# interactiveaudiolab/ppgs

Measured on AMD Instinct MI355X. Metric: PPG frames/sec (whole node), mel repr, batch=32x1000 frames, higher is better.
Workload: dtype bf16; 1 GPU; configs[1]: mel representation, batch=32 x 1000 frames per GPU, audio resident in HBM -> (32,40,1000) fp32 posteriors in HBM; batch=32, frames=1000, per_gpu_batches=1, parallelism=utterance-sharded x1, no data-path collective

## Files before the change

### ppgs_amd/csrc/ppg_engine.hip

```cpp
#include "ppg_pack.h"

#include <stdarg.h>

using namespace ppg;

static thread_local std::string g_error;

int ppg::fail_message(int code, const char* fmt, ...) {
    char buf[512];
    va_list ap;
    va_start(ap, fmt);
    vsnprintf(buf, sizeof(buf), fmt, ap);
    va_end(ap);
    g_error = buf;
    return code;
}

PpgEngine::~PpgEngine() {
    (void)hipSetDevice(device);
#ifdef PPG_TIMING_BUILD
    dump_timing_stamps(this);
#endif
    for (void* p : {(void*)d_overflow, (void*)head_dbg, (void*)ffn_dbg, (void*)attn_dbg, (void*)lin_dbg}) if (p) (void)hipFree(p);
    for (auto& kv : plans) if (kv.second->buf) (void)hipFree(kv.second->buf);
// ... 335 lines not shown
        HIP_OK(hipMemset(e->attn_dbg, 0, 512 + 4096 * 32));
    }
#endif
#ifdef PPG_H32_TIMING
    if (getenv("PPGS_AMD_H32_TIMING")) {
        HIP_OK(hipMalloc(reinterpret_cast<void**>(&e->head_dbg), 512));
        HIP_OK(hipMemset(e->head_dbg, 0, 512));
    }
#endif
#ifdef PPG_FFN_TIMING
    if (getenv("PPGS_AMD_FFN_TIMING")) {
        HIP_OK(hipMalloc(reinterpret_cast<void**>(&e->ffn_dbg), 2048));
        HIP_OK(hipMemset(e->ffn_dbg, 0, 2048));
    }
#endif
    if (e->ffn_nt < 0 || e->ffn_nt > 3) e->ffn_nt = 0;
    {
        hipDeviceProp_t prop;
        if (hipGetDeviceProperties(&prop, device) == hipSuccess && prop.multiProcessorCount > 0)
            e->num_cus = prop.multiProcessorCount;
    }

    int rc;
    if ((rc = pk.upload_f32(wts->position_encoding, (size_t)cfg->max_positions * H, 0, &e->pe))) return rc;
    {
        const float* w = wts->input_weight;
        const int Cp = e->Cp;
        rc = pk.matrix(H, 5 * Cp, H, e->in_total_groups * e->KG,
                       [&](int row, int k) { const int h = pair_row(row), tap = k / Cp, c = k % Cp; return c < C ? w[((size_t)h * C + c) * 5 + tap] : 0.f; },
                       &e->w_in);
        if (rc) return rc;
        if ((rc = pk.upload_f32(wts->input_bias, H, 0, &e->b_in))) return rc;
    }
    const int RB = H / 128, KS = H / 16;
    auto wave_row = [&](int w, int rb, int ln) { return 32 * RB * w + 32 * rb + phi(ln & 31); };
    if (e->head32) {
        const float* w = wts->input_weight;
        const int KSI = 5 * e->Cp / 16, frags = 4 * RB * KSI;
        rc = pk.image(frags + 1, [&](int f, int ln, int j) {
            if (f >= frags) return 0.f;
            const int ks = f % KSI, rb = (f / KSI) % RB, wv = f / (KSI * RB);
            const int tap = ks / (e->Cp / 16), c = frag_k(ks % (e->Cp / 16), ln, j);
            return c < C ? w[((size_t)wave_row(wv, rb, ln) * C + c) * 5 + tap] : 0.f;
        }, &e->win_img);
        if (rc) return rc;
    }
    {
        const float* w = wts->output_weight;
        rc = pk.matrix(cfg->output_channels, 5 * H, 48, e->out_total_groups * e->KG,
                       [&](int n, int k) { const int tap = k / H, c = k % H; return w[((size_t)n * H + c) * 5 + tap]; },
                       &e->w_out);
        if (rc) return rc;
        if ((rc = pk.upload_f32(wts->output_bias, cfg->output_channels, 48, &e->b_out))) return rc;
    }
    e->layers.resize(L);
    const float qscale = (float)(1.4426950408889634 / sqrt((double)dh));
    std::vector<float> in_w((size_t)3 * H * H), in_b((size_t)3 * H);
    for (int l = 0; l < L; ++l) {
        DevLayer& d = e->layers[l];
        for (size_t i = 0; i < in_w.size(); ++i) in_w[i] = wts->in_proj_weight[l][i] * (i < (size_t)H * H ? qscale : 1.0f);
        for (int i = 0; i < 3 * H; ++i) in_b[i] = wts->in_proj_bias[l][i] * (i < H ? qscale : 1.0f);
        const float *wq = in_w.data(), *wo = wts->out_proj_weight[l], *w1 = wts->linear1_weight[l], *w2 = wts->linear2_weight[l];
        auto paired = [&](const float* w, int rows, int cols, bool pair_rows, bool pair_k, char** dst) {
            return pk.matrix(rows, cols, rows, cols, [&](int r, int c) { return w[(size_t)(pair_rows ? pair_row(r) : r) * cols + (pair_k ? pair_row(c) : c)]; }, dst);
        };
        if ((rc = paired(wq, 3 * H, H, true, false, &d.wqkv))) return rc;
        if ((rc = paired(wo, H, H, true, false, &d.wo))) return rc;
        if ((rc = paired(w1, F, H, false, false, &d.w1))) return rc;
        if ((rc = paired(w2, H, F, true, false, &d.w2))) return rc;
        d.wqkvk = d.wqkv;
        d.w1k = d.w1;
        if (pk.fmt == Fmt::F32) {
            if ((rc = paired(wq, 3 * H, H, true, true, &d.wqkvk))) return rc;
            if ((rc = paired(w1, F, H, false, true, &d.w1k))) return rc;
        }
        {
            const bool bf = pk.fmt != Fmt::F32;
            rc = pk.matrix(H, F, H, F,
                           [&](int row, int c) {
                               const int r = pair_row(row);
                               if (!bf) return w2[(size_t)r * F + c];
                               const int grp = c / 32, s = c % 32, g = s / 8, ee = (s % 8) / 4, rr = s % 4;
                               return w2[(size_t)r * F + grp * 32 + 16 * ee + 4 * g + rr];
                           },
                           &d.w2p);
            if (rc) return rc;
        }
        auto qkv_row = [&](int w, int st, int ln) {
            const int rb = st % RB, kind = st / RB;
            return kind < 2 ? kind * H + wave_row(w, rb, ln) : 2 * H + pair_row(32 * RB * w + 32 * rb + (ln & 31));
        };
        if (e->layer32) {
            rc = pk.image(4 * RB * KS, [&](int f, int ln, int j) {
                const int ks = f % KS, rb = (f / KS) % RB, w = f / (KS * RB);
                return wo[(size_t)wave_row(w, rb, ln) * H + frag_k(ks, ln, j)];
            }, &d.wo_img);
            if (rc) return rc;
            rc = pk.image(F / 128 * 4 * KS, [&](int f, int ln, int j) {
                const int ks = f % KS, w = (f / KS) & 3, ch = f / (KS * 4);
                return w1[(size_t)(ch * 128 + 32 * w + (ln & 31)) * H + panel_k(ks, ln, j)];
            }, &d.w1_img);
            if (rc) return rc;
            rc = pk.image(F / 128 * 4 * RB * 8, [&](int f, int ln, int j) {
                const int ks = f & 7, rb = (f >> 3) % RB, w = (f / (8 * RB)) & 3, ch = f / (8 * RB * 4);
                return w2[(size_t)wave_row(w, rb, ln) * F + ch * 128 + hidden_k(ks, ln, j)];
            }, &d.w2_img);
// ... 218 lines not shown
        if (r.form[l] == kLayer32) {
            Timed t(e, PPG_K_FFN, r.s);
            Layer32Args a{};
            a.ao = r.ao; a.wo_img = d.wo_img; a.w1_img = d.w1_img; a.w2_img = d.w2_img;
            a.bo = d.bo; a.g1 = d.g1; a.e1 = d.e1; a.b1 = d.b1; a.b2 = d.b2; a.g2 = d.g2; a.e2 = d.e2;
            a.X = r.X; a.Xb = r.Xb; a.M = M; a.F = F; a.H = H; a.dbg = l == 0 ? e->ffn_dbg : nullptr;
            a.debug_mode = e->l32_debug;
            a.x_half = e->x16;
            a.sub_tiles = r.sub32;
            a.write_x = l + 1 < c.num_layers;
            if (qkv_next) {
                qkv_tail(&a, r, e->layers[l + 1].wq_img, e->layers[l + 1].bqkv);
                a.Xb = nullptr;
            }
            LAUNCH_OK(ppg::launch_layer32(prec, a, r.s), "layer32");
            return PPG_OK;
        }
        if (!r.fuse_op && !(r.form[l] == kFfn32x2 && e->ffn32x2 >= 2)) {
            Timed t(e, PPG_K_OUTPROJ_LN, r.s);
            LinearArgs a = outproj_ln_args(e, rows, d, r.ao);
            if (l == 0 && e->lin_dbg_class == PPG_K_OUTPROJ_LN) a.dbg = e->lin_dbg;
            LAUNCH_OK(ppg::launch_linear(prec, EPI_RESLN, H / 16, r.lnt_ln, a, 1, r.s), "out-proj+LN");
        }
        Timed t(e, PPG_K_FFN, r.s);
        if (r.form[l] == kFfn32x2) {
            Ffn32X2Args a{};
            a.xb = r.Xb; a.X = r.X; a.xb_out = r.Xb; a.w1_img = d.w1x_img; a.w2_img = d.w2x_img;
            a.b1 = d.b1; a.b2 = d.b2; a.g2 = d.g2; a.e2 = d.e2; a.M = M; a.F = F; a.H = H;
            if (e->ffn32x2 >= 2) { a.ao = r.ao; a.wo_img = d.wox_img; a.bo = d.bo; a.g1 = d.g1; a.e1 = d.e1; }
            a.dbg = l == 0 ? e->ffn_dbg : nullptr;
            if (qkv_next) qkv_tail(&a, r, e->layers[l + 1].wqx_img, e->layers[l + 1].bqkv);
            LAUNCH_OK(ppg::launch_ffn32x2(a, r.s), "ffn32x2");
        } else if (r.form[l] == kFfnFused) {
            FfnArgs a = ffn_args(e, rows, d, r.ws.ffn_splits, reinterpret_cast<float*>(r.base + r.ws.part));
            a.dbg = l == 0 ? e->ffn_dbg : nullptr;
            if (r.fuse_op) ffn_fuse_outproj(&a, d, r.ao);
            if (qkv_next) ffn_fuse_qkv(&a, rows, e->layers[l + 1], r.qk, r.vt, r.ws.vt_ld);
            LAUNCH_OK(ppg::launch_ffn(prec, a, r.ws.ffn_nt, r.s), "ffn");
        } else {
            LinearArgs a = gemm_args(e, rows, r.act_x, H, d.w1, d.b1, F);
            a.out_rows = r.hid; a.out_ld = F;
            LAUNCH_OK(ppg::launch_linear(prec, EPI_RELU, 16, r.lnt, a, F / 256, r.s), "ffn1");
            LinearArgs b = gemm_args(e, rows, r.hid, F, d.w2, d.b2, H);
            b.gamma = d.g2; b.beta = d.e2;
            LAUNCH_OK(ppg::launch_linear(prec, EPI_RESLN, H / 16, r.lnt_ln, b, 1, r.s), "ffn2+LN");
        }
        return PPG_OK;
    };

    auto enqueue_outconv = [&](const Route& r) -> int {
        Timed t(e, PPG_K_OUTCONV_SOFTMAX, r.s);
        LinearArgs a = outconv_args(e, rows_of(r), r.act_x, out, frames, softmax);
        if (e->lin_dbg_class == PPG_K_OUTCONV_SOFTMAX) a.dbg = e->lin_dbg;
        if (e->outconv && ppg::outconv_supported(prec, a)) LAUNCH_OK(ppg::launch_outconv(prec, a, r.s), "out-conv+softmax");
        else LAUNCH_OK(ppg::launch_linear(prec, EPI_OUTCONV, 3, r.lnt_ln, a, 1, r.s), "out-conv+softmax");
        return PPG_OK;
    };

    std::vector<Route> routes;
    routes.reserve(plan.groups.size());
    for (size_t gi = 0; gi < plan.groups.size(); ++gi) routes.push_back(route_of(plan.groups[gi], gi == 0 ? s : e->side_streams[gi - 1]));
    return fork_join(s, e->ev_fork, e->side_streams.data(), e->ev_join.data(), routes.size() - 1, [&]() -> int {
        for (int seg = 0; seg < c.num_layers + 2; ++seg)
            for (const Route& r : routes) {
                const int rc = seg == 0 ? enqueue_head(r) : seg <= c.num_layers ? enqueue_layer(r, seg - 1) : enqueue_outconv(r);
                if (rc) return rc;
            }
        return PPG_OK;
    });
}

int ppg_engine_nonfinite(PpgEngine* e, int clear, int* flag) {
    if (!e || !flag) return fail(PPG_EINVAL, "null argument");
    if (!e->d_overflow) { *flag = 0; return PPG_OK; }
    std::lock_guard<std::mutex> lock(e->mu);
    HIP_OK(hipSetDevice(e->device));
    unsigned value = 0;
    HIP_OK(hipMemcpy(&value, e->d_overflow, sizeof(value), hipMemcpyDeviceToHost));
    if (value && clear) HIP_OK(hipMemset(e->d_overflow, 0, sizeof(value)));
    *flag = (int)value;
    return PPG_OK;
}

int ppg_engine_pipelines(const PpgEngine* e, int tokens) {
    if (!e || tokens < 0) return 0;
    return group_count(e, tokens);
}

int ppg_engine_profile(PpgEngine* e, int enable) {
    if (!e) return fail(PPG_EINVAL, "null engine");
    e->profiling = (unsigned)enable;
    if (enable) (void)hipSetDevice(e->device);
    for (int cls = 0; enable && cls < PPG_K_COUNT; ++cls) {
        if (!(e->profiling & (1u << cls))) continue;
        while (e->events[cls].size() < 32) {
            EventPair p;
            if (hipEventCreateWithFlags(&p.a, kTimingEventFlags) != hipSuccess || hipEventCreateWithFlags(&p.b, kTimingEventFlags) != hipSuccess) break;
            e->events[cls].push_back(p);
        }
    }
    return PPG_OK;
}

int ppg_engine_profile_reset(PpgEngine* e) {
    if (!e) return fail(PPG_EINVAL, "null engine");
    for (auto& u : e->events_used) u = 0;
    for (auto& q : e->launch_seq) q = 0;
// ... 17 lines not shown
```

### ppgs_amd/csrc/ppg_head32.hip

```cpp
#include "ppg_layer32.h"

namespace {

constexpr int HID = 256;
constexpr int CP = 96;
constexpr int ROWB = 208;
constexpr int HALO = 2;
constexpr int KSI = 5 * CP / 16;
constexpr int KSH = KSI / 2;

template <int K0, int TBN>
struct OffIn {
    static constexpr int at(int i) {
        const int ks = K0 + i / TBN, tb = i % TBN;
        return (32 * tb + ks / (CP / 16)) * ROWB + (ks % (CP / 16)) * 32;
    }
};

template <class P, int TBS>
__global__ __launch_bounds__(256) __attribute__((amdgpu_waves_per_eu(1, 1))) void head32_kernel(Head32Args a) {
    using G = Geo<HID, TBS>;
    constexpr int RB = G::RB, KS = G::KS, TB = G::TBN, TOKS = G::TOKS;
    constexpr int TBT = tile_blocks(HID);
    constexpr bool SUB = TBS != TBT;
    constexpr int NSUB = (TBT + TBS - 1) / TBS;
    static_assert(RB == 2 && KSI % 2 == 0, "two row blocks per wave, two register sets");
    extern __shared__ __attribute__((aligned(16))) char smem[];
    const int tid = threadIdx.x;
    if ((int)blockIdx.x >= a.tiles * NSUB) {
        for (int job = blockIdx.x - a.tiles * NSUB; job <= a.nwin + 1; job += gridDim.x - a.tiles * NSUB) {
            if (job == a.nwin + 1) {
                for (int i = tid; i < a.qk_slack_bytes / 16; i += 256) reinterpret_cast<uint4*>(a.qk_slack)[i] = make_uint4(0u, 0u, 0u, 0u);
            } else if (job == a.nwin) {
                const int chunks = (a.vt_ld - a.vt_tokens) * 2 / 16;
                for (int i = tid; i < a.vt_rows * chunks; i += 256) {
                    const int r = i / chunks, c = i - r * chunks;
                    *reinterpret_cast<uint4*>(a.vt_out + ((size_t)r * a.vt_ld + a.vt_tokens) * 2 + c * 16) = make_uint4(0u, 0u, 0u, 0u);
                }
            } else {
                const PpgWindow w = a.win[job];
                const int r16 = (w.frames + 15) & ~15, r32 = (w.frames + 31) & ~31;
                if (r32 != r16) {
                    const int col = w.vt_off + r32 - 32;
                    for (int i = tid; i < a.vt_rows * 4; i += 256) {
                        const int r = i >> 2, g = i & 3;
                        *reinterpret_cast<uint2*>(a.vt_out + ((size_t)r * a.vt_ld + col + 8 * g + 4) * 2) = make_uint2(0u, 0u);
                    }
                }
            }
        }
        return;
    }
    const int lane = tid & 63;
    const int wave = __builtin_amdgcn_readfirstlane(tid >> 6);
    const int tok = lane & 31, hh = lane >> 5;
    const int tile = SUB ? (int)blockIdx.x / NSUB : (int)blockIdx.x;
    const int tb0 = SUB ? ((int)blockIdx.x % NSUB) * TBS : 0;
    const int nblk = SUB ? min(TBS, TBT - tb0) : TBS;
    const int m0 = tile * (32 * TBT) + 32 * tb0;
    const uint32_t lds0 = lds_addr32(smem);
    const uint32_t voff = lane * 16;
    const uint32_t pb0 = lds0 + G::L_ACT + lane * 16;
    const int fbase = 32 * RB * wave;
    char* rows = smem + G::L_H;
    static_assert((TOKS + 2 * HALO) * ROWB <= TB * 8 * 1024, "the gathered tile fits the h region");
    float* bq_lds = reinterpret_cast<float*>(smem + G::L_BQ);

#ifdef PPG_H32_TIMING
    auto pstamp = [&](int k) {
        if (!SUB && a.dbg && blockIdx.x == 0 && lane == 0) a.dbg[wave * 16 + k] = __builtin_amdgcn_s_memtime();
    };
#else
    auto pstamp = [&](int) {};
#endif
    pstamp(0);
    u32x4 w1f[16], w2f[16];
    auto load16 = [&](u32x4 (&wf)[16], const char* base) {
        [&]<int... K>(std::integer_sequence<int, K...>) { (gload_frag<K>(wf[K], voff, base), ...); }(std::make_integer_sequence<int, 16>{});
    };
    const char* wimg = a.win_img + ((size_t)wave * RB * KSI) * 1024;
    const char* wq0 = a.wq_img + ((size_t)wave * 3 * RB * KS) * 1024;
    load16(w1f, wimg);
    load16(w2f, wimg + (size_t)KSI * 1024);

    if (tid < TOKS + 2 * HALO && !(PPG_DBG(a) & 4)) {
        const int m = m0 - HALO + tid;
        int frame = -1;
        size_t base = 0;
        if (m >= 0) {
            const TokMeta tm = tok_meta(a.blk_win, a.win, m, a.M);
            if (tm.w >= 0 && tm.tt < tm.frames) {
                const PpgWindow w = a.win[tm.w];
                frame = w.chunked ? max(w.start + tm.tt - a.overlap, 0) : tm.tt;
                base = (size_t)w.item * a.C * a.T;
            }
        }
        uint32_t* dst = reinterpret_cast<uint32_t*>(rows + tid * ROWB);
        const int C = a.C;
        const bool row_live = frame >= 0;
        const size_t off = base + (size_t)max(frame, 0);
        float v[CP];
        if (a.dtype == PPG_DTYPE_F16) {
            const __half* src = reinterpret_cast<const __half*>(a.feats) + off;
#pragma unroll
            for (int c = 0; c < CP; ++c) v[c] = __half2float(src[(size_t)min(c, C - 1) * a.T]);
// ... 18 lines not shown
        live[t] = tm.w >= 0 && tm.tt < tm.frames;
        valid[t] = live[t] && tm.tt < tm.valid;
        tt[t] = live[t] ? tm.tt : 0;
        dlo[t] = live[t] ? -tm.tt : -HALO;
        dhi[t] = live[t] ? tm.frames - 1 - tm.tt : HALO;
        unsigned bits = 0;
#pragma unroll
        for (int tap = 0; tap < 5; ++tap)
            if (__any(tap - HALO < dlo[t] || tap - HALO > dhi[t])) bits |= 1u << tap;
        edge[t] = bits;
    }

    pstamp(2);
    f32x16 yacc[RB][TB];
    const f32x16 zero = {0.f, 0.f, 0.f, 0.f, 0.f, 0.f, 0.f, 0.f, 0.f, 0.f, 0.f, 0.f, 0.f, 0.f, 0.f, 0.f};
    const uint32_t rb0 = lds0 + G::L_H + (uint32_t)(tok * ROWB + hh * 16);
    float4 pe[TB][4];
    auto load_pe = [&](int rb) {
#pragma unroll
        for (int t = 0; t < TB; ++t)
#pragma unroll
            for (int q = 0; q < 4; ++q)
                pe[t][q] = *reinterpret_cast<const float4*>(a.pe + (size_t)tt[t] * HID + fbase + 32 * rb + 16 * hh + 4 * q);
    };
    auto round = [&](auto r_tag, auto after_wait) {
        constexpr int R = decltype(r_tag)::value;
        vm_wait_all(w1f);
        vm_wait_all(w2f);
        after_wait();
        if constexpr (R == 0) __syncthreads();
        stream<OffIn<KSH * R, TB>, KSH * TB, 6>(rb0, rb0, [&](auto ic, const u32x4& bf) {
            constexpr int i = decltype(ic)::value;
            constexpr int ksl = i / TB, tb = i % TB, tap = (KSH * R + ksl) / (CP / 16);
            u32x4 b = bf;
            if constexpr (tap != HALO) {
                if (edge[tb] & (1u << tap)) {
                    const bool ok = tap - HALO >= dlo[tb] && tap - HALO <= dhi[tb];
                    b = u32x4{ok ? bf.x : 0u, ok ? bf.y : 0u, ok ? bf.z : 0u, ok ? bf.w : 0u};
                }
            }
            if constexpr (R == 0 && ksl == 0) {
                yacc[0][tb] = P::mma32(w1f[0], b, zero);
                yacc[1][tb] = P::mma32(w2f[0], b, zero);
            } else {
                yacc[0][tb] = P::mma32(w1f[ksl], b, yacc[0][tb]);
                yacc[1][tb] = P::mma32(w2f[ksl], b, yacc[1][tb]);
            }
            if constexpr (R == 0 && tb == TB - 1) {
                gload_frag<ksl>(w1f[ksl], voff, wimg + (size_t)KSH * 1024);
                gload_frag<ksl>(w2f[ksl], voff, wimg + (size_t)(KSI + KSH) * 1024);
            }
        });
    };
    if (!(PPG_DBG(a) & 1)) round(std::integral_constant<int, 0>{}, [] {});
    else __syncthreads();
    pstamp(3);
    if (!(PPG_DBG(a) & 1)) round(std::integral_constant<int, 1>{}, [&] { load_pe(0); });
    else load_pe(0);

    pstamp(4);
    float* xt = a.X + ((size_t)tile * 4 + wave) * (TBT * RB * 4 * 256) + lane * 4;
    char* xh = reinterpret_cast<char*>(a.X) + ((size_t)tile * 4 + wave) * (TBT * RB * 2 * 1024) + lane * 16;
    auto emit = [&](auto rb_tag) {
        constexpr int rb = decltype(rb_tag)::value;
        const int f0 = fbase + 32 * rb + 16 * hh;
        float4 bias[4], pv[TB][4];
#pragma unroll
        for (int q = 0; q < 4; ++q) bias[q] = *reinterpret_cast<const float4*>(a.b_in + f0 + 4 * q);
#pragma unroll
        for (int t = 0; t < TB; ++t)
#pragma unroll
            for (int q = 0; q < 4; ++q) pv[t][q] = pe[t][q];
        if constexpr (rb + 1 < RB) load_pe(rb + 1);
#pragma unroll
        for (int t = 0; t < TB; ++t) {
            f32x16 y;
#pragma unroll
            for (int q = 0; q < 4; ++q) {
                y[4 * q + 0] = live[t] ? pv[t][q].x + (valid[t] ? yacc[rb][t][4 * q + 0] + bias[q].x : 0.f) : 0.f;
                y[4 * q + 1] = live[t] ? pv[t][q].y + (valid[t] ? yacc[rb][t][4 * q + 1] + bias[q].y : 0.f) : 0.f;
                y[4 * q + 2] = live[t] ? pv[t][q].z + (valid[t] ? yacc[rb][t][4 * q + 2] + bias[q].z : 0.f) : 0.f;
                y[4 * q + 3] = live[t] ? pv[t][q].w + (valid[t] ? yacc[rb][t][4 * q + 3] + bias[q].w : 0.f) : 0.f;
                if (!a.x_half && t < nblk)
                    *reinterpret_cast<float4*>(xt + (((tb0 + t) * RB + rb) * 4 + q) * 256) = make_float4(y[4 * q + 0], y[4 * q + 1], y[4 * q + 2], y[4 * q + 3]);
            }
            if (a.x_half && t < nblk) {
#pragma unroll
                for (int s2 = 0; s2 < 2; ++s2)
                    *reinterpret_cast<u32x4*>(xh + (((tb0 + t) * RB + rb) * 2 + s2) * 1024) = u32x4{pack_f16x2(y[8 * s2 + 0], y[8 * s2 + 1]), pack_f16x2(y[8 * s2 + 2], y[8 * s2 + 3]),
                                                                                      pack_f16x2(y[8 * s2 + 4], y[8 * s2 + 5]), pack_f16x2(y[8 * s2 + 6], y[8 * s2 + 7])};
            }
            panel_store<P, HID, TBS>(pb0, wave, t, rb, y);
        }
    };
    emit(std::integral_constant<int, 0>{});
    emit(std::integral_constant<int, 1>{});
    pstamp(5);
    load16(w1f, wq0);
    vm_wait_all(w1f);
    pstamp(6);

    Layer32Args la{};
    la.wq_img = a.wq_img; la.qk_out = a.qk_out; la.vt_out = a.vt_out; la.vt_ld = a.vt_ld;
    la.blk_win = a.blk_win; la.win = a.win; la.M = a.M; la.H = HID;
    if (!(PPG_DBG(a) & 2)) qkv_tail<P, HID, TBS>(la, smem, m0, w1f, w2f, nblk);
    asm volatile("s_waitcnt vmcnt(0)" ::: "memory");
    pstamp(7);
}

}

namespace ppg {

hipError_t launch_head32(int precision, const Head32Args& a, hipStream_t s) {
    if (a.H != HID || a.C > CP || a.M <= 0 || a.tiles != (a.M + 32 * tile_blocks(HID) - 1) / (32 * tile_blocks(HID))) return hipErrorInvalidValue;
    auto launch = [&](auto kern, auto geo, int subs) {
        using G = decltype(geo);
        const size_t lds = G::L_B1;
        const dim3 grid(a.tiles * subs + std::min(a.nwin + 2, 32));
        static ppg::LdsLimit limit;
        const hipError_t e = limit.ensure(reinterpret_cast<const void*>(kern), lds);
        if (e != hipSuccess) return e;
        hipLaunchKernelGGL(kern, grid, dim3(256), lds, s, a);
        return hipGetLastError();
    };
    constexpr int T5 = tile_blocks(HID);
    if (precision == PPG_PRECISION_BF16) return a.sub_tiles ? launch(head32_kernel<PrecBF16, 2>, Geo<HID, 2>{}, 3) : launch(head32_kernel<PrecBF16, T5>, Geo<HID>{}, 1);
    if (precision == PPG_PRECISION_FP16) return a.sub_tiles ? launch(head32_kernel<PrecF16, 2>, Geo<HID, 2>{}, 3) : launch(head32_kernel<PrecF16, T5>, Geo<HID>{}, 1);
    return hipErrorInvalidValue;
}

}
```

### ppgs_amd/csrc/ppg_host.h

```cpp
#pragma once

#include "ppg_launch.h"

#include <limits.h>
#include <math.h>
#include <stdio.h>
#include <string.h>

#include <map>
#include <memory>
#include <mutex>
#include <string>
#include <vector>

namespace ppg {

int fail_message(int code, const char* fmt, ...);
inline int (&fail)(int, const char*, ...) = fail_message;

#define HIP_OK(expr) \
    do { if (hipError_t e_ = (expr); e_ != hipSuccess) return fail(PPG_EDEVICE, "%s failed: %s", #expr, hipGetErrorString(e_)); } while (0)
#define LAUNCH_OK(expr, what) \
    do { if (hipError_t he_ = (expr); he_ != hipSuccess) return fail(PPG_EDEVICE, "%s: %s", what, hipGetErrorString(he_)); } while (0)

// ... 105 lines not shown
    size_t xw, x, xb, qk, vt, ao, hid, part, total;
    int ffn_nt, ffn_splits;
    int vt_ld, qk_rows;
};

}

struct PpgEngine {
    PpgConfig cfg{};
    int device = 0;
    int sz = 4;
    int KG = 16;
    int Cp = 0;
    int in_groups_per_tap = 0, in_total_groups = 0;
    int out_groups_per_tap = 0, out_total_groups = 0;
    int head_dim = 0;
    int ffn_nt = 0;
    int lin_nt = 0;
    int num_cus = 256;
    bool ffn_fused = true;
    bool qkv_fused = true;
    int ffn_split_max = 0;
    int ffn_splits_forced = 0;
    bool ffn_mixed = true;
    bool op_fused = true;
    bool attn_xcd = true;
    bool outconv = true;
    bool head32 = true;
    char* win_img = nullptr;
    int attn_narrow = 1;
    unsigned* d_overflow = nullptr;
    int ffn32x2 = 3;
    bool subtile = true;
    bool x16 = false;
    bool layer32 = true;
    bool ffn_split = true;
    int num_streams = 2;
    std::vector<hipStream_t> side_streams;
    bool stream_one_pass = false;
    int stream_min_rows = 128;
    hipEvent_t ev_fork = nullptr;
    std::vector<hipEvent_t> ev_join;
    int l32_debug = 0, h32_debug = 0;
    unsigned long long* ffn_dbg = nullptr;
    unsigned long long* head_dbg = nullptr;
    unsigned long long* attn_dbg = nullptr;
    unsigned long long* lin_dbg = nullptr;
    int lin_dbg_class = -1;
    ppg::Packer pack;
    bool split() const { return pack.split(); }
    float* pe = nullptr;
    char* w_in = nullptr; float* b_in = nullptr;
    char* w_out = nullptr; float* b_out = nullptr;
    std::vector<ppg::DevLayer> layers;
    std::map<std::string, std::unique_ptr<ppg::DevPlan>> plans;
    uint64_t plan_stamp = 0;
    std::vector<ppg::RetiredBuf> retired;
    ppg::StageSlot stage[4];
    int stage_next = 0;
    std::mutex mu;
    unsigned profiling = 0;
    std::vector<ppg::EventPair> events[PPG_K_COUNT];
    size_t events_used[PPG_K_COUNT] = {0};
    int profile_stride = 1;
    size_t launch_seq[PPG_K_COUNT] = {0};

    ~PpgEngine();
};

namespace ppg {

#if defined(PPG_FFN_TIMING) || defined(PPG_ATTN_TIMING) || defined(PPG_H32_TIMING) || defined(PPG_LIN_TIMING)
#define PPG_TIMING_BUILD 1
void dump_timing_stamps(const PpgEngine* e);
#endif

int choose_nt(int num_cus, int forced_nt, int M, int max_nt);
inline int ffn_chunks(int hidden, int ffn, int sz) { return ffn / (32768 / (hidden * sz)); }
constexpr size_t kLdsBytes = 163840;
inline size_t ffn_lds_bytes(int hidden, int ffn, int rows) { return 131072 + (size_t)ffn * 4 + (size_t)rows * hidden * 4; }
inline bool ffn_fits(int hidden, int ffn, bool op) { return ffn_lds_bytes(hidden, ffn, op ? 9 : 6) <= kLdsBytes; }
inline bool ffn_mixed_fits(int hidden, int ffn) { return ffn_lds_bytes(hidden, ffn, 6) + 16384 <= kLdsBytes; }
Workspace layout(const PpgEngine* e, int tokens, int vt_tokens);
inline int stream_query_tile(int head_dim) { return head_dim == 128 ? attn_query_tile(head_dim) / 2 : attn_query_tile(head_dim); }

template <class Body>
int fork_join(hipStream_t s, hipEvent_t fork, const hipStream_t* side, const hipEvent_t* join, size_t n, Body&& body) {
    if (n == 0) return body();
    const int rc = [&]() -> int {
        HIP_OK(hipEventRecord(fork, s));
        for (size_t i = 0; i < n; ++i) HIP_OK(hipStreamWaitEvent(side[i], fork, 0));
        return body();
    }();
    if (rc != PPG_OK) {
        for (size_t i = 0; i < n; ++i) {
            (void)hipEventRecord(join[i], side[i]);
            (void)hipStreamWaitEvent(s, join[i], 0);
        }
        return rc;
    }
    for (size_t i = 0; i < n; ++i) {
        HIP_OK(hipEventRecord(join[i], side[i]));
        HIP_OK(hipStreamWaitEvent(s, join[i], 0));
    }
    return PPG_OK;
}
// ... 102 lines not shown
```

### ppgs_amd/csrc/ppg_launch.h

```cpp
#pragma once

#include <algorithm>
#include <cstdlib>
#include <hip/hip_runtime.h>

#include "ppg_device.h"

namespace ppg {

inline int env_switch(const char* name, int dflt) {
    const char* s = getenv(name);
    return s ? atoi(s) : dflt;
}
#ifdef PPG_EXPERIMENT_SWITCHES
inline int env_experiment(const char* name, int dflt) { return env_switch(name, dflt); }
inline bool env_experiment_set(const char* name) { return getenv(name) != nullptr; }
#else
inline int env_experiment(const char*, int dflt) { return dflt; }
inline bool env_experiment_set(const char*) { return false; }
#endif

int attn_query_tile(int head_dim);

hipError_t launch_gather(int precision, const GatherArgs& a, hipStream_t s);
hipError_t launch_fill(float* p, size_t n, float v, hipStream_t s);

hipError_t launch_linear(int precision, int epi, int nb, int nt, const LinearArgs& a, int ypasses, hipStream_t s);
constexpr int kFfnMixedTiling = 5;
hipError_t launch_ffn(int precision, const FfnArgs& a, int nt, hipStream_t s);
hipError_t launch_attn(int precision, const AttnArgs& a, int nitems, int heads, int head_dim, hipStream_t s);
hipError_t launch_layer32(int precision, const Layer32Args& a, hipStream_t s);
hipError_t launch_head32(int precision, const Head32Args& a, hipStream_t s);
hipError_t launch_gemm32(int precision, const Gemm32Args& a, hipStream_t s);
hipError_t launch_posconv(int precision, const PosConvArgs& a, int batch, hipStream_t s);
hipError_t launch_ffn32x2(const Ffn32X2Args& a, hipStream_t s);
int ffn32x2_tokens();
bool ffn32x2_supported(int H, int F);
bool outconv_supported(int precision, const LinearArgs& a);
hipError_t launch_outconv(int precision, const LinearArgs& a, hipStream_t s);
int layer32_tokens(int hidden);
int layer32_max_ffn(int hidden);
hipError_t launch_w2v2_layer0(int precision, const float* audio, int batch, long samples, long frames, int rows_per_item,
                              const float* w0, const float* gamma, const float* beta, double* moments, float2* scale_shift,
                              char* out, hipStream_t s);
hipError_t launch_w2v2_layernorm(int precision, int H, const float* in32, const char* in16, const float* gamma, const float* beta,
                                 long rows, int T_in, int R_out, float eps, float* out32, char* out16, hipStream_t s);
hipError_t launch_w2v2_output(int precision, const char* rows, int batch, int rows_per_item, long frames, float* out, hipStream_t s);

constexpr int kFrontendFrames = 16;
constexpr int kMelSteps = 8;
constexpr int kMelSegment = 5;

struct LdsLimit {
    size_t bytes[32] = {};
    hipError_t ensure(const void* kernel, size_t lds) {
        int device = 0;
        if (hipGetDevice(&device) != hipSuccess || device < 0 || device >= 32) device = 0;
        if (bytes[device] >= lds) return hipSuccess;
        const hipError_t e = hipFuncSetAttribute(kernel, hipFuncAttributeMaxDynamicSharedMemorySize, (int)lds);
        if (e == hipSuccess) bytes[device] = lds;
        return e;
    }
};

struct FrontendTables {
    const float* hann;
    const float2* twiddle;
    const void* mel_img;
    const int4* mel_prog;
    unsigned long long* dbg;
};

hipError_t launch_frontend(const FrontendTables& tb, const float* audio, int batch, int samples,
                           void* spec, void* mel, hipStream_t s);

struct FrontendStreamItem {
    int lo;
    int hi;
    int cbase;
    int split;
    int frames;
    int keep;
    int cur;
    int pad;
};
constexpr int kFrontendStreamItems = 64;
struct FrontendStreamArgs {
    const float* chunk;
    float* carry;
    long chunk_pitch;
    int cap;
    int item0;
// ... 8 lines not shown
```

### ppgs_amd/csrc/ppg_outconv.hip

```cpp
#include "ppg_lds.h"
#include "ppg_launch.h"

#include <utility>

#ifdef PPG_ONLY_BF16
#define PPG_OTHER_PRECISIONS 0
#else
#define PPG_OTHER_PRECISIONS 1
#endif

namespace {

constexpr int OT = 64;
constexpr int HALO = 2;
constexpr int NB = 3;
constexpr int KTAP = 256;
constexpr int KSTEPS = 5 * KTAP / 32;
constexpr int WROW = 5 * KTAP * 2;
constexpr int WP = WROW + 32;
constexpr int TP = KTAP * 2 + 32;
constexpr int L_TILE = NB * 16 * WP;
constexpr int LDS_BYTES = L_TILE + (OT + 2 * HALO) * TP;
static_assert(LDS_BYTES <= 160 * 1024, "one workgroup per CU");
constexpr int ROW_CHUNKS = KTAP * 2 / 16;
constexpr int STG = ((OT + 2 * HALO) * ROW_CHUNKS + 255) / 256;

template <class P>
__global__ __launch_bounds__(256) void outconv_kernel(LinearArgs a) {
    extern __shared__ __attribute__((aligned(16))) char smem[];
    const int tid = threadIdx.x;
    const int lane = tid & 63;
    const int wave = __builtin_amdgcn_readfirstlane(tid >> 6);
    const int idx = lane & 15, g = lane >> 4;

    float bias[NB][4];
#pragma unroll
    for (int nb = 0; nb < NB; ++nb) {
        const float4 bv = *reinterpret_cast<const float4*>(a.bias + nb * 16 + 4 * g);
        bias[nb][0] = bv.x; bias[nb][1] = bv.y; bias[nb][2] = bv.z; bias[nb][3] = bv.w;
    }

    const int ntiles = (a.M + OT - 1) / OT;
    u32x4 stg[STG];
    auto fetch = [&](int tile) {
#pragma unroll
        for (int j = 0; j < STG; ++j) {
            const int i = min(tid + 256 * j, (OT + 2 * HALO) * ROW_CHUNKS - 1);
            const int r = i / ROW_CHUNKS, piece = i - r * ROW_CHUNKS;
            const int m = min(max(tile * OT - HALO + r, 0), a.M - 1);
            stg[j] = *reinterpret_cast<const u32x4*>(a.act + (size_t)m * a.lda_bytes + piece * 16);
        }
    };
    auto stash = [&]() {
#pragma unroll
        for (int j = 0; j < STG; ++j) {
            const int i = tid + 256 * j;
            if (i < (OT + 2 * HALO) * ROW_CHUNKS) {
                const int r = i / ROW_CHUNKS, piece = i - r * ROW_CHUNKS;
                *reinterpret_cast<u32x4*>(smem + L_TILE + r * TP + piece * 16) = stg[j];
            }
        }
    };
    struct Meta { TokMeta tm; int keep_lo, keep_hi, out_frame, item; };
    auto lookup_block = [&](int tile) {
        const int m = tile * OT + 16 * wave + idx;
        return m < a.M ? a.blk_win[m >> 4] : -1;
    };
    auto lookup_window = [&](int tile, int w) {
        Meta r;
        const PpgWindow win = a.win[max(w, 0)];
        r.tm.w = w;
        r.tm.tt = w >= 0 ? tile * OT + 16 * wave + idx - win.tok_off : 0;
        r.tm.frames = w >= 0 ? win.frames : 0;
        r.tm.valid = w >= 0 ? win.valid : 0;
        r.keep_lo = win.keep_lo; r.keep_hi = win.keep_hi; r.out_frame = win.out_frame; r.item = win.item;
        return r;
    };
    Meta cur{};
    int wcur = -1;
    if ((int)blockIdx.x < ntiles) { fetch(blockIdx.x); wcur = lookup_block(blockIdx.x); }

    constexpr int WPIECES = NB * 16 * (WROW / 16), WBATCH = 15;
    static_assert(WPIECES == 2 * WBATCH * 256, "two batches");
#pragma unroll
    for (int half = 0; half < 2; ++half) {
        u32x4 wv[WBATCH];
#pragma unroll
        for (int j = 0; j < WBATCH; ++j) {
            const int i = tid + 256 * (half * WBATCH + j);
            const int row = i / (WROW / 16), piece = i - row * (WROW / 16);
            wv[j] = *reinterpret_cast<const u32x4*>(a.W + (size_t)row * a.total_groups * 64 + piece * 16);
        }
        if (half == 1 && (int)blockIdx.x < ntiles) cur = lookup_window(blockIdx.x, wcur);
#pragma unroll
        for (int j = 0; j < WBATCH; ++j) {
            const int i = tid + 256 * (half * WBATCH + j);
            const int row = i / (WROW / 16), piece = i - row * (WROW / 16);
            *reinterpret_cast<u32x4*>(smem + row * WP + piece * 16) = wv[j];
        }
    }
    const uint32_t lds0 = lds_addr(smem);
    uint32_t waddr[NB];
#pragma unroll
    for (int nb = 0; nb < NB; ++nb) waddr[nb] = lds0 + (uint32_t)((nb * 16 + idx) * WP + g * 16);
    const uint32_t xaddr = lds0 + (uint32_t)(L_TILE + (16 * wave + idx) * TP + g * 16);
    const int step = gridDim.x;
    if ((int)blockIdx.x < ntiles) {
        stash();
        if ((int)blockIdx.x + step < ntiles) fetch(blockIdx.x + step);
    }
    __syncthreads();
    for (int tile = blockIdx.x; tile < ntiles; tile += step) {
        const bool more = tile + step < ntiles;
        const int wnext = more ? lookup_block(tile + step) : -1;
        const TokMeta tm = cur.tm;
        unsigned taps_ok = 0;
#pragma unroll
        for (int d = 0; d < 5; ++d) {
            const int st = tm.tt + d - HALO;
            if (tm.w >= 0 && st >= 0 && st < tm.frames) taps_ok |= 1u << d;
        }
        const bool edge = __any(taps_ok != 0x1fu);

        f32x4 acc[NB];
#pragma unroll
        for (int nb = 0; nb < NB; ++nb) acc[nb] = f32x4{0.f, 0.f, 0.f, 0.f};
        constexpr int NFRAG = 4 * KSTEPS, RING = 12;
        u32x4 ring[RING];
        auto issue = [&](auto ic) {
            constexpr int i = decltype(ic)::value;
            constexpr int ks = i / 4, j = i % 4, per_tap = KTAP / 32;
            if constexpr (j == 0) ds_read_b128_asm<(ks / per_tap) * TP + (ks % per_tap) * 64>(ring[i % RING], xaddr);
            else ds_read_b128_asm<ks * 64>(ring[i % RING], waddr[j - 1]);
        };
        u32x4 bcur = u32x4{0u, 0u, 0u, 0u};
        [&]<int... I>(std::integer_sequence<int, I...>) { (issue(std::integral_constant<int, I>{}), ...); }(std::make_integer_sequence<int, RING>{});
        [&]<int... I>(std::integer_sequence<int, I...>) {
            ([&] {
                constexpr int ks = I / 4, j = I % 4, tap = ks / (KTAP / 32);
                constexpr int behind = NFRAG - 1 - I < RING - 1 ? NFRAG - 1 - I : RING - 1;
                lgkm_wait<behind>(ring[I % RING]);
                if constexpr (j == 0) {
                    bcur = ring[I % RING];
                    if (edge && !((taps_ok >> tap) & 1u)) bcur = u32x4{0u, 0u, 0u, 0u};
                } else {
                    P::mma(acc[j - 1], ring[I % RING], bcur);
                }
                if constexpr (I + RING < NFRAG) issue(std::integral_constant<int, I + RING>{});
            }(), ...);
        }(std::make_integer_sequence<int, NFRAG>{});

        __syncthreads();
        if (more) stash();
        Meta nxt{};
        if (more) nxt = lookup_window(tile + step, wnext);
        const bool live = tm.w >= 0 && tm.tt < tm.frames;
        const bool valid = live && tm.tt < tm.valid;
        float v[NB][4];
        float mx = -INFINITY, chk = 0.f;
#pragma unroll
        for (int nb = 0; nb < NB; ++nb)
#pragma unroll
            for (int r = 0; r < 4; ++r) {
                const int n = nb * 16 + 4 * g + r;
                v[nb][r] = valid ? acc[nb][r] + bias[nb][r] : 0.f;
                if (n < a.out_C) mx = fmaxf(mx, v[nb][r]);
                if (n < a.out_C) chk = fmaf(v[nb][r], 0.f, chk);
            }
        if (chk != chk && a.overflow) atomicOr(a.overflow, 1u);
        if (a.softmax) {
            mx = wave_max_g(mx);
            float sum = 0.f;
#pragma unroll
            for (int nb = 0; nb < NB; ++nb)
#pragma unroll
                for (int r = 0; r < 4; ++r) {
                    const int n = nb * 16 + 4 * g + r;
                    const float e = (n < a.out_C) ? expf(v[nb][r] - mx) : 0.f;
                    v[nb][r] = e;
                    sum += e;
                }
            sum = wave_sum_g(sum);
            const float inv = 1.0f / sum;
#pragma unroll
            for (int nb = 0; nb < NB; ++nb)
#pragma unroll
                for (int r = 0; r < 4; ++r) v[nb][r] *= inv;
        }
        if (live) {
            if (tm.tt >= cur.keep_lo && tm.tt < cur.keep_hi) {
                const int frame = cur.out_frame + (tm.tt - cur.keep_lo);
                float* o = a.out + (size_t)cur.item * a.out_C * a.out_T + frame;
#pragma unroll
                for (int nb = 0; nb < NB; ++nb)
#pragma unroll
                    for (int r = 0; r < 4; ++r) {
                        const int n = nb * 16 + 4 * g + r;
                        if (n < a.out_C) o[(size_t)n * a.out_T] = v[nb][r];
                    }
            }
        }
        if (tile + 2 * step < ntiles) fetch(tile + 2 * step);
        __syncthreads();
        cur = nxt;
    }
}

}

namespace ppg {

bool outconv_supported(int precision, const LinearArgs& a) {
    return precision != PPG_PRECISION_FP32 && a.taps == 5 && a.lda_bytes == KTAP * 2 && a.real_groups == 5 * KTAP / 32 &&
           a.total_groups * 64 >= WROW && a.N == NB * 16 && a.out_C <= NB * 16;
}

hipError_t launch_outconv(int precision, const LinearArgs& a, hipStream_t s) {
    if (!outconv_supported(precision, a)) return hipErrorInvalidValue;
    static LdsLimit limit[2];
    static int cus = 0;
    if (cus == 0) {
        int dev = 0;
        if (hipGetDevice(&dev) != hipSuccess ||
            hipDeviceGetAttribute(&cus, hipDeviceAttributeMultiprocessorCount, dev) != hipSuccess || cus <= 0)
            cus = 256;
    }
    const int ntiles = (a.M + OT - 1) / OT;
    const int rounds = (ntiles + cus - 1) / cus;
    const int grid = (ntiles + rounds - 1) / rounds;
    if (precision == PPG_PRECISION_BF16) {
        const hipError_t e = limit[0].ensure(reinterpret_cast<const void*>(outconv_kernel<PrecBF16>), LDS_BYTES);
        if (e != hipSuccess) return e;
        hipLaunchKernelGGL(outconv_kernel<PrecBF16>, dim3(grid), dim3(256), LDS_BYTES, s, a);
    } else {
#if PPG_OTHER_PRECISIONS
        const hipError_t e = limit[1].ensure(reinterpret_cast<const void*>(outconv_kernel<PrecF16>), LDS_BYTES);
        if (e != hipSuccess) return e;
        hipLaunchKernelGGL(outconv_kernel<PrecF16>, dim3(grid), dim3(256), LDS_BYTES, s, a);
#else
        return hipErrorInvalidValue;
#endif
    }
    return hipGetLastError();
}

}
```

### ppgs_amd/csrc/ppg_pack.h

```cpp
#pragma once

#include "ppg_host.h"

namespace ppg {

inline int phi(int rho) { return 16 * ((rho >> 2) & 1) + 4 * (rho >> 3) + (rho & 3); }
inline int frag_k(int ks, int ln, int j) { return 16 * ks + 8 * (ln >> 5) + j; }
inline int panel_k(int ks, int ln, int j) { return 32 * (ks >> 1) + 16 * (ln >> 5) + 8 * (ks & 1) + j; }
inline int hidden_k(int ks, int ln, int j) { return 32 * (ks >> 1) + 16 * (ks & 1) + 8 * (j >> 2) + 4 * (ln >> 5) + (j & 3); }
inline void split_f16(float v, uint16_t* hi, uint16_t* lo) { *hi = host_f16(v); *lo = host_f16(v - host_f16_to_f32(*hi)); }

inline int Packer::upload(const void* src, size_t bytes, void** dst) {
    void* p = nullptr;
    HIP_OK(hipMalloc(&p, std::max<size_t>(bytes, 16)));
    allocs.push_back(p);
    HIP_OK(hipMemcpy(p, src, bytes, hipMemcpyHostToDevice));
    *dst = p;
    return PPG_OK;
}

inline int Packer::upload_f32(const float* src, size_t n, size_t n_pad, float** dst) {
    std::vector<float> tmp(std::max(n, n_pad), 0.f);
    memcpy(tmp.data(), src, n * sizeof(float));
    return upload(tmp.data(), tmp.size() * sizeof(float), reinterpret_cast<void**>(dst));
}

template <class F>
int Packer::matrix(Fmt as, int rows, int cols, int rows_pad, int cols_pad, F get, char** dst) {
    const size_t n = (size_t)rows_pad * cols_pad;
    if (as == Fmt::F16X2) {
        if (cols_pad % 32) return fail(PPG_EINVAL, "split-precision operand rows are multiples of 32 elements (%d)", cols_pad);
        std::vector<uint16_t> tmp(2 * n, 0);
        for (int r = 0; r < rows; ++r)
            for (int c = 0; c < cols; ++c) {
                const size_t at = ((size_t)r * cols_pad + (c / 32) * 32) * 2 + (c % 32);
                split_f16(get(r, c), &tmp[at], &tmp[at + 32]);
            }
        return upload(tmp.data(), n * 4, reinterpret_cast<void**>(dst));
    }
    if (as != Fmt::F32) {
        std::vector<uint16_t> tmp(n, 0);
        for (int r = 0; r < rows; ++r)
            for (int c = 0; c < cols; ++c) tmp[(size_t)r * cols_pad + c] = as == Fmt::F16 ? host_f16(get(r, c)) : host_bf16(get(r, c));
        return upload(tmp.data(), n * 2, reinterpret_cast<void**>(dst));
    }
    std::vector<float> tmp(n, 0.f);
    for (int r = 0; r < rows; ++r)
        for (int c = 0; c < cols; ++c) tmp[(size_t)r * cols_pad + c] = get(r, c);
    return upload(tmp.data(), n * 4, reinterpret_cast<void**>(dst));
}

template <class F>
int Packer::image(int frags, F get, char** dst) {
    return matrix(frags * 64, 8, frags * 64, 8, [&](int r, int j) { return get(r >> 6, r & 63, j); }, dst);
}

template <class F>
int Packer::image_hilo(int groups, F get, char** dst) {
    std::vector<uint16_t> tmp((size_t)groups * 32 * 512);
    for (int g = 0; g < groups; ++g)
        for (int f = 0; f < 16; ++f)
            for (int ln = 0; ln < 64; ++ln)
                for (int j = 0; j < 8; ++j) {
                    const size_t at = ((size_t)g * 32 + f) * 512 + ln * 8 + j;
                    split_f16(get(g, f, ln, j), &tmp[at], &tmp[at + 16 * 512]);
                }
    return upload(tmp.data(), tmp.size() * 2, reinterpret_cast<void**>(dst));
}

template <class F>
int gemm32_image(Packer& pk, int N, int K, F get, char** dst) {
    const int chunks = K / 128;
    return pk.image((N / 256) * 4 * chunks * 16, [&](int f, int ln, int j) {
        const int ks = f & 7, rb = (f >> 3) & 1, c = (f >> 4) % chunks, wv = ((f >> 4) / chunks) & 3, p = (f >> 4) / chunks / 4;
        const int n0 = 256 * p + 64 * wv + 32 * rb;
        return get(n0 + phi(ln & 31), n0 + (ln & 31), 128 * c + frag_k(ks, ln, j));
    }, dst);
}

}
```

Measured before the change: 47.15 million frames/s.

## Pre-pack out-conv weights into LDS image, DMA them, fold zeroing into head tiles

Builds at load time a packed out-conv weight image that matches the kernel's LDS layout and pitch. The out-conv kernel then fills LDS with global-to-LDS DMA copies of 1 KB pieces instead of staging through registers, and sizes its grid by dividing CUs among concurrent pipelines. The head32 kernel no longer launches extra blocks for scratch zeroing; each tile block does that zeroing inside its first round. This aims to cut weight-load latency and extra blocks, at the cost of more work in the head tiles and tighter coupling between the host packer and the kernel layout.

```diff
diff --git a/ppgs_amd/csrc/ppg_engine.hip b/ppgs_amd/csrc/ppg_engine.hip
--- a/ppgs_amd/csrc/ppg_engine.hip
+++ b/ppgs_amd/csrc/ppg_engine.hip
@@ -411,6 +411,9 @@
                        &e->w_out);
         if (rc) return rc;
         if ((rc = pk.upload_f32(wts->output_bias, cfg->output_channels, 48, &e->b_out))) return rc;
+        if (e->outconv && e->sz == 2 && H == 256 && cfg->output_channels <= ppg::kOutconvRows &&
+            (rc = outconv_image(pk, w, cfg->output_channels, H, &e->w_out_img)))
+            return rc;
     }
     e->layers.resize(L);
     const float qscale = (float)(1.4426950408889634 / sqrt((double)dh));
@@ -735,7 +738,7 @@
         Timed t(e, PPG_K_OUTCONV_SOFTMAX, r.s);
         LinearArgs a = outconv_args(e, rows_of(r), r.act_x, out, frames, softmax);
         if (e->lin_dbg_class == PPG_K_OUTCONV_SOFTMAX) a.dbg = e->lin_dbg;
-        if (e->outconv && ppg::outconv_supported(prec, a)) LAUNCH_OK(ppg::launch_outconv(prec, a, r.s), "out-conv+softmax");
+        if (e->w_out_img && ppg::outconv_supported(prec, a)) LAUNCH_OK(ppg::launch_outconv(prec, a, e->w_out_img, r.sub32 ? 1 : (int)plan.groups.size(), r.s), "out-conv+softmax");
         else LAUNCH_OK(ppg::launch_linear(prec, EPI_OUTCONV, 3, r.lnt_ln, a, 1, r.s), "out-conv+softmax");
         return PPG_OK;
     };
diff --git a/ppgs_amd/csrc/ppg_head32.hip b/ppgs_amd/csrc/ppg_head32.hip
--- a/ppgs_amd/csrc/ppg_head32.hip
+++ b/ppgs_amd/csrc/ppg_head32.hip
@@ -27,8 +27,11 @@
     static_assert(RB == 2 && KSI % 2 == 0, "two row blocks per wave, two register sets");
     extern __shared__ __attribute__((aligned(16))) char smem[];
     const int tid = threadIdx.x;
-    if ((int)blockIdx.x >= a.tiles * NSUB) {
-        for (int job = blockIdx.x - a.tiles * NSUB; job <= a.nwin + 1; job += gridDim.x - a.tiles * NSUB) {
+    const int zjob = blockIdx.x;
+    int zframes = 0, zvt_off = 0;
+    if (zjob < a.nwin) { zframes = a.win[zjob].frames; zvt_off = a.win[zjob].vt_off; }
+    auto zero_scratch = [&]() {
+        for (int job = zjob; job <= a.nwin + 1; job += gridDim.x) {
             if (job == a.nwin + 1) {
                 for (int i = tid; i < a.qk_slack_bytes / 16; i += 256) reinterpret_cast<uint4*>(a.qk_slack)[i] = make_uint4(0u, 0u, 0u, 0u);
             } else if (job == a.nwin) {
@@ -38,10 +41,11 @@
                     *reinterpret_cast<uint4*>(a.vt_out + ((size_t)r * a.vt_ld + a.vt_tokens) * 2 + c * 16) = make_uint4(0u, 0u, 0u, 0u);
                 }
             } else {
-                const PpgWindow w = a.win[job];
-                const int r16 = (w.frames + 15) & ~15, r32 = (w.frames + 31) & ~31;
+                const int frames = job == zjob ? zframes : a.win[job].frames;
+                const int vt_off = job == zjob ? zvt_off : a.win[job].vt_off;
+                const int r16 = (frames + 15) & ~15, r32 = (frames + 31) & ~31;
                 if (r32 != r16) {
-                    const int col = w.vt_off + r32 - 32;
+                    const int col = vt_off + r32 - 32;
                     for (int i = tid; i < a.vt_rows * 4; i += 256) {
                         const int r = i >> 2, g = i & 3;
                         *reinterpret_cast<uint2*>(a.vt_out + ((size_t)r * a.vt_ld + col + 8 * g + 4) * 2) = make_uint2(0u, 0u);
@@ -49,8 +53,7 @@
                 }
             }
         }
-        return;
-    }
+    };
     const int lane = tid & 63;
     const int wave = __builtin_amdgcn_readfirstlane(tid >> 6);
     const int tok = lane & 31, hh = lane >> 5;
@@ -175,8 +178,8 @@
             }
         });
     };
-    if (!(PPG_DBG(a) & 1)) round(std::integral_constant<int, 0>{}, [] {});
-    else __syncthreads();
+    if (!(PPG_DBG(a) & 1)) round(std::integral_constant<int, 0>{}, [&] { zero_scratch(); });
+    else { zero_scratch(); __syncthreads(); }
     pstamp(3);
     if (!(PPG_DBG(a) & 1)) round(std::integral_constant<int, 1>{}, [&] { load_pe(0); });
     else load_pe(0);
@@ -240,7 +243,7 @@
     auto launch = [&](auto kern, auto geo, int subs) {
         using G = decltype(geo);
         const size_t lds = G::L_B1;
-        const dim3 grid(a.tiles * subs + std::min(a.nwin + 2, 32));
+        const dim3 grid(a.tiles * subs);
         static ppg::LdsLimit limit;
         const hipError_t e = limit.ensure(reinterpret_cast<const void*>(kern), lds);
         if (e != hipSuccess) return e;
diff --git a/ppgs_amd/csrc/ppg_host.h b/ppgs_amd/csrc/ppg_host.h
--- a/ppgs_amd/csrc/ppg_host.h
+++ b/ppgs_amd/csrc/ppg_host.h
@@ -181,6 +181,7 @@
     float* pe = nullptr;
     char* w_in = nullptr; float* b_in = nullptr;
     char* w_out = nullptr; float* b_out = nullptr;
+    char* w_out_img = nullptr;
     std::vector<ppg::DevLayer> layers;
     std::map<std::string, std::unique_ptr<ppg::DevPlan>> plans;
     uint64_t plan_stamp = 0;
diff --git a/ppgs_amd/csrc/ppg_launch.h b/ppgs_amd/csrc/ppg_launch.h
--- a/ppgs_amd/csrc/ppg_launch.h
+++ b/ppgs_amd/csrc/ppg_launch.h
@@ -36,8 +36,9 @@
 hipError_t launch_ffn32x2(const Ffn32X2Args& a, hipStream_t s);
 int ffn32x2_tokens();
 bool ffn32x2_supported(int H, int F);
+constexpr int kOutconvRows = 48, kOutconvPitchPad = 32;
 bool outconv_supported(int precision, const LinearArgs& a);
-hipError_t launch_outconv(int precision, const LinearArgs& a, hipStream_t s);
+hipError_t launch_outconv(int precision, const LinearArgs& a, const char* w_image, int pipelines, hipStream_t s);
 int layer32_tokens(int hidden);
 int layer32_max_ffn(int hidden);
 hipError_t launch_w2v2_layer0(int precision, const float* audio, int batch, long samples, long frames, int rows_per_item,
diff --git a/ppgs_amd/csrc/ppg_outconv.hip b/ppgs_amd/csrc/ppg_outconv.hip
--- a/ppgs_amd/csrc/ppg_outconv.hip
+++ b/ppgs_amd/csrc/ppg_outconv.hip
@@ -66,9 +66,8 @@
         const int m = tile * OT + 16 * wave + idx;
         return m < a.M ? a.blk_win[m >> 4] : -1;
     };
-    auto lookup_window = [&](int tile, int w) {
+    auto window_meta = [&](int tile, int w, const PpgWindow& win) {
         Meta r;
-        const PpgWindow win = a.win[max(w, 0)];
         r.tm.w = w;
         r.tm.tt = w >= 0 ? tile * OT + 16 * wave + idx - win.tok_off : 0;
         r.tm.frames = w >= 0 ? win.frames : 0;
@@ -76,39 +75,41 @@
         r.keep_lo = win.keep_lo; r.keep_hi = win.keep_hi; r.out_frame = win.out_frame; r.item = win.item;
         return r;
     };
-    Meta cur{};
+    auto lookup_window = [&](int tile, int w) { return window_meta(tile, w, a.win[max(w, 0)]); };
+
+    const uint32_t lds0 = lds_addr(smem);
+    constexpr int WDMA = (L_TILE + 1023) / 1024, WTURNS = (WDMA + 3) / 4;
+    static_assert(L_TILE >= 1024 && L_TILE % 16 == 0, "whole 16-byte lanes");
+    auto weights_dma = [&](auto i0, auto i1) {
+        [&]<int... I>(std::integer_sequence<int, I...>) {
+            ([&] {
+                constexpr int i = decltype(i0)::value + I;
+                const int piece = 4 * i + wave;
+                if (4 * i + 3 < WDMA - 1) {
+                    glds16_saddr(a.W + piece * 1024, (uint32_t)(lane * 16), lds0 + (uint32_t)(piece * 1024));
+                } else if (piece < WDMA) {
+                    const int at = min(piece * 1024, L_TILE - 1024);
+                    glds16_saddr(a.W + at, (uint32_t)(lane * 16), lds0 + (uint32_t)at);
+                }
+            }(), ...);
+        }(std::make_integer_sequence<int, decltype(i1)::value - decltype(i0)::value>{});
+    };
+    const bool first = (int)blockIdx.x < ntiles;
     int wcur = -1;
-    if ((int)blockIdx.x < ntiles) { fetch(blockIdx.x); wcur = lookup_block(blockIdx.x); }
-
-    constexpr int WPIECES = NB * 16 * (WROW / 16), WBATCH = 15;
-    static_assert(WPIECES == 2 * WBATCH * 256, "two batches");
-#pragma unroll
-    for (int half = 0; half < 2; ++half) {
-        u32x4 wv[WBATCH];
-#pragma unroll
-        for (int j = 0; j < WBATCH; ++j) {
-            const int i = tid + 256 * (half * WBATCH + j);
-            const int row = i / (WROW / 16), piece = i - row * (WROW / 16);
-            wv[j] = *reinterpret_cast<const u32x4*>(a.W + (size_t)row * a.total_groups * 64 + piece * 16);
-        }
-        if (half == 1 && (int)blockIdx.x < ntiles) cur = lookup_window(blockIdx.x, wcur);
-#pragma unroll
-        for (int j = 0; j < WBATCH; ++j) {
-            const int i = tid + 256 * (half * WBATCH + j);
-            const int row = i / (WROW / 16), piece = i - row * (WROW / 16);
-            *reinterpret_cast<u32x4*>(smem + row * WP + piece * 16) = wv[j];
-        }
-    }
-    const uint32_t lds0 = lds_addr(smem);
+    if (first) fetch(blockIdx.x);
+    weights_dma(std::integral_constant<int, 0>{}, std::integral_constant<int, WTURNS / 2>{});
+    if (first) wcur = lookup_block(blockIdx.x);
+    const PpgWindow wfirst = a.win[max(wcur, 0)];
+    weights_dma(std::integral_constant<int, WTURNS / 2>{}, std::integral_constant<int, WTURNS>{});
+    Meta cur = window_meta(blockIdx.x, wcur, wfirst);
     uint32_t waddr[NB];
 #pragma unroll
     for (int nb = 0; nb < NB; ++nb) waddr[nb] = lds0 + (uint32_t)((nb * 16 + idx) * WP + g * 16);
     const uint32_t xaddr = lds0 + (uint32_t)(L_TILE + (16 * wave + idx) * TP + g * 16);
     const int step = gridDim.x;
-    if ((int)blockIdx.x < ntiles) {
-        stash();
-        if ((int)blockIdx.x + step < ntiles) fetch(blockIdx.x + step);
-    }
+    if ((int)blockIdx.x < ntiles) stash();
+    asm volatile("s_waitcnt vmcnt(0)" ::: "memory");
+    if ((int)blockIdx.x + step < ntiles) fetch(blockIdx.x + step);
     __syncthreads();
     for (int tile = blockIdx.x; tile < ntiles; tile += step) {
         const bool more = tile + step < ntiles;
@@ -215,8 +216,12 @@
            a.total_groups * 64 >= WROW && a.N == NB * 16 && a.out_C <= NB * 16;
 }
 
-hipError_t launch_outconv(int precision, const LinearArgs& a, hipStream_t s) {
-    if (!outconv_supported(precision, a)) return hipErrorInvalidValue;
+static_assert(NB * 16 == kOutconvRows && WP == WROW + kOutconvPitchPad, "the engine's image is this kernel's LDS layout");
+
+hipError_t launch_outconv(int precision, const LinearArgs& args, const char* w_image, int pipelines, hipStream_t s) {
+    if (!outconv_supported(precision, args) || !w_image || pipelines < 1) return hipErrorInvalidValue;
+    LinearArgs a = args;
+    a.W = w_image;
     static LdsLimit limit[2];
     static int cus = 0;
     if (cus == 0) {
@@ -226,7 +231,8 @@
             cus = 256;
     }
     const int ntiles = (a.M + OT - 1) / OT;
-    const int rounds = (ntiles + cus - 1) / cus;
+    const int share = std::max(1, cus / pipelines);
+    const int rounds = (ntiles + share - 1) / share;
     const int grid = (ntiles + rounds - 1) / rounds;
     if (precision == PPG_PRECISION_BF16) {
         const hipError_t e = limit[0].ensure(reinterpret_cast<const void*>(outconv_kernel<PrecBF16>), LDS_BYTES);
diff --git a/ppgs_amd/csrc/ppg_pack.h b/ppgs_amd/csrc/ppg_pack.h
--- a/ppgs_amd/csrc/ppg_pack.h
+++ b/ppgs_amd/csrc/ppg_pack.h
@@ -68,6 +68,22 @@
     return upload(tmp.data(), tmp.size() * 2, reinterpret_cast<void**>(dst));
 }
 
+inline std::vector<uint16_t> outconv_image_host(Fmt as, const float* w, int out_channels, int H) {
+    const size_t pitch = (size_t)5 * H + kOutconvPitchPad / 2;
+    std::vector<uint16_t> img(kOutconvRows * pitch, 0);
+    for (int n = 0; n < out_channels && n < kOutconvRows; ++n)
+        for (int tap = 0; tap < 5; ++tap)
+            for (int c = 0; c < H; ++c) {
+                const float v = w[((size_t)n * H + c) * 5 + tap];
+                img[n * pitch + (size_t)tap * H + c] = as == Fmt::F16 ? host_f16(v) : host_bf16(v);
+            }
+    return img;
+}
+inline int outconv_image(Packer& pk, const float* w, int out_channels, int H, char** dst) {
+    const std::vector<uint16_t> img = outconv_image_host(pk.fmt, w, out_channels, H);
+    return pk.upload(img.data(), img.size() * 2, reinterpret_cast<void**>(dst));
+}
+
 template <class F>
 int gemm32_image(Packer& pk, int N, int K, F get, char** dst) {
     const int chunks = K / 128;
```

Result: no change. 47.11 million frames/s (-0.1%).
